# mattiaskvist/yolo-v1

Hardware: AMD Instinct MI355X
Metric: images/sec at 448x448, forward (YOLOv1Backbone + FC head) (higher is better)
Workload: dtype bf16; 1 GPU; BASELINE.json configs[1]: batch=64/GPU 448x448 forward-only, YOLOv1Backbone + FC head, 1xMI355X per rank; global_batch=64, per_gpu_batch=64, weights=random init (torch default, seed 0), parallelism=single

## Files before the change

include/yolo_hip.h:

```cpp
#ifndef YOLO_HIP_H
#define YOLO_HIP_H

#include <stddef.h>
#include <stdint.h>

#ifdef __cplusplus
extern "C" {
#endif

#define YOLO_HIP_ABI_VERSION 2

#define YOLO_E_ARG (-1)
#define YOLO_E_UNSUPPORTED (-2)

typedef void *yolo_stream_t;

int yolo_hip_abi_version(void);
const char *yolo_hip_last_error(void);
int yolo_debug_stamps(void *buf, int k_iter);
int yolo_stream_create(int low, yolo_stream_t *out);


int yolo_decode(const float *pred, int N, int S, int B, int C, double conf_thr,
                double *rec, int32_t *counts, yolo_stream_t stream);
// ... 52 lines not shown
#define YOLO_EPI_BIAS_LRELU 2
#define YOLO_EPI_MUL_DLRELU 3

#define YOLO_EPI_BIAS_ADD_LRELU 4

int yolo_igemm(const yolo_igemm_desc *d, const void *in_bf16, const void *w_bf16 ,
               const float *bias, const void *aux_bf16, void *out, yolo_stream_t stream);
int yolo_igemm_finish(const yolo_igemm_desc *d, const float *acc, const float *bias, const void *aux_bf16,
                      void *out_bf16, yolo_stream_t stream);

typedef struct yolo_wgrad_desc {
    int64_t P;
    int32_t dy_px_stride, x_px_stride;
    int32_t Cout, Cin;
    int32_t KH, KW, pad;
    int64_t x_row_stride;
    int32_t split;
    int32_t accumulate;
    int32_t variant;
    int32_t geo_W, geo_H, geo_img_slots, geo_row_slots, geo_px_slots, geo_slot0;
    double *dw_sumsq;
    float *slabs;
    int64_t slab_floats;
} yolo_wgrad_desc;

int yolo_wgrad_slab_floats(const yolo_wgrad_desc *d, long *floats);
int yolo_wgrad(const yolo_wgrad_desc *d, const void *x_bf16, const void *dy_bf16,
               float *dw_packed, float *db, yolo_stream_t stream);

typedef struct yolo_pool_desc {
    int32_t N, H, W, C;
    int32_t in_halo, out_halo;
} yolo_pool_desc;
int yolo_maxpool3s2_fwd(const yolo_pool_desc *d, const void *x_bf16, void *y_bf16, yolo_stream_t stream);
int yolo_maxpool3s2_bwd(const yolo_pool_desc *d, const void *x_bf16, const void *dy_bf16, void *dx_bf16, int dx_halo,
                        yolo_stream_t stream);
int yolo_maxpool2_fwd(const yolo_pool_desc *d, const void *x_bf16, void *y_bf16, yolo_stream_t stream);
int yolo_maxpool2_bwd_lrelu(const yolo_pool_desc *d, const void *yfull_bf16, const void *dpool_bf16,
                            float slope, void *dz_bf16, yolo_stream_t stream);
int yolo_maxpool2_bwd_codes(const yolo_pool_desc *d, const void *ypool_bf16, const void *codes_u16, const void *dpool_bf16,
                            float slope, void *dz_bf16, yolo_stream_t stream);


int yolo_nchw_f32_to_nhwc_bf16(const float *x, int N, int C, int H, int W, void *y, int Cpad,
                               int halo_lo, int halo_hi, yolo_stream_t stream);
int yolo_nhwc_bf16_to_nchw_f32(const void *x, int N, int C, int H, int W, int halo, float *y, yolo_stream_t stream);
int yolo_nhwc_bf16_to_nchw_bf16(const void *x, int N, int C, int H, int W, int halo, void *y, yolo_stream_t stream);

int yolo_pack_conv_weight(const float *w_oihw, int Cout, int Cin, int KH, int KW, int Cinp, int KWp,
                          void *w_fwd_bf16, void *w_dgrad_bf16, yolo_stream_t stream);
int yolo_pack_fc_weight(const float *w, int O, int C, int HW, void *w_fwd_bf16, void *w_t_bf16, yolo_stream_t stream);
int yolo_pack_fc_weight_blocked(const float *w, int O, long K, void *w_panels_bf16, yolo_stream_t stream);
int yolo_pack_fc_weight_blocked_hwc(const float *w, int O, int C, int HW, void *w_panels_bf16, yolo_stream_t stream);
int yolo_unpack_conv_wgrad(const float *dw_packed, int Cout, int Cin, int KH, int KW, int Cinp, int KWp,
                           float *dw_oihw, int accumulate, yolo_stream_t stream);
int yolo_conv_stem7_fwd(const void *x_nhwc4_bf16, const void *w_packed_bf16, const float *bias, int N, int Ho, int Wo,
                        long x_img_stride, int x_row_stride, float slope, int pool2, void *out_bf16,
                        long out_img_stride, int out_row_stride, int out_off, void *out_full_bf16,
                        long full_img_stride, int full_row_stride, int full_off, yolo_stream_t stream);
int yolo_conv_stem7_fwd_f32(const float *x_nchw_f32, const void *w_packed_bf16, const float *bias, int N, int H, int W, float slope,
                            int pool2, void *out_bf16, long out_img_stride, int out_row_stride, int out_off, void *out_full_bf16,
                            long full_img_stride, int full_row_stride, int full_off, yolo_stream_t stream);
int yolo_wgrad_stem7(const void *x_nhwc4_bf16, const void *dy_bf16, int N, int Ho, int Wo, long x_img_stride,
                     int x_row_stride, long dy_img_stride, int dy_row_stride, int dy_off, float *dw_oihw,
                     float *db, float *scratch, long scratch_elems, yolo_stream_t stream);
int yolo_wgrad_stem7_pooled(const void *x_nhwc4_bf16, const void *y_full_bf16, int N, int Ho, int Wo, long x_img_stride,
                            int x_row_stride, long y_img_stride, int y_row_stride, int y_off, const void *dpool_bf16,
                            long dp_img_stride, int dp_row_stride, int dp_off, float slope, float *dw_oihw, float *db,
                            float *scratch, long scratch_elems, yolo_stream_t stream);
int yolo_wgrad_stem7_codes(const void *x_nhwc4_bf16, const void *y_pooled_bf16, const void *codes_u16, int N, int Ho, int Wo,
                           long x_img_stride, int x_row_stride, const void *dpool_bf16, long dp_img_stride, int dp_row_stride,
                           int dp_off, float slope, float *dw_oihw, float *db, float *scratch, long scratch_elems,
                           yolo_stream_t stream);
#define YOLO_PACK_MAX 32
typedef struct yolo_conv_pack_item {
    const float *w;
    void *w_fwd_bf16;
    void *w_dgrad_bf16;
    int Cout, Cin, KH, KW;
} yolo_conv_pack_item;
typedef struct yolo_conv_unpack_item {
    const float *dw_packed;
    float *dw_oihw;
    int Cout, Cin, KH, KW;
} yolo_conv_unpack_item;
int yolo_pack_conv_weights_multi(const yolo_conv_pack_item *items, int count, yolo_stream_t stream);
int yolo_unpack_conv_wgrads_multi(const yolo_conv_unpack_item *items, int count, yolo_stream_t stream);
int yolo_im2col_rows(const void *x_bf16, long x_img_stride, int x_row_stride, int x_px_stride, int stride,
                     int KH, int seg, int N, int Ho, int Wo, int out_halo, void *xcol_bf16, yolo_stream_t stream);
int yolo_transpose_f32_to_bf16(const float *x, int R, int Ccols, void *y_bf16, int ld, yolo_stream_t stream);
int yolo_transpose_bf16(const void *x_bf16, int R, int Ccols, int ldx, void *y_bf16, int ldy, yolo_stream_t stream);
int yolo_fc_dgrad_to_nhwc(const float *dxT, int N, int C, int H, int W, int halo, const void *y_act_bf16,
                          float slope, void *g_bf16, yolo_stream_t stream);
int yolo_cast_f32_to_bf16(const float *x, long n, void *y_bf16, yolo_stream_t stream);
int yolo_cast_bf16_to_f32(const void *x_bf16, long n, float *y, yolo_stream_t stream);
int yolo_bias_lrelu_rows(const float *x, const float *bias, int R, int Ccols, float slope,
                         void *y_bf16, float *y_f32, yolo_stream_t stream);
int yolo_bias_lrelu_rows_slabs(const float *x, int slabs, const float *bias, int R, int Ccols, float slope,
                               void *y_bf16, float *y_f32, yolo_stream_t stream);

int yolo_scale_rows_to_bf16(const float *x, const unsigned char *mask, float scale, const void *act_bf16, float slope,
                            int R, int Cc, int ld, void *y_bf16, yolo_stream_t stream);
int yolo_dropout_bf16(const void *x_bf16, const unsigned char *mask, float scale, long n, void *y_bf16, yolo_stream_t stream);

int yolo_sumsq_f32(const float *g, long n, double *acc, yolo_stream_t stream);
int yolo_adam_step(float *p, const float *g, float *exp_avg, float *exp_avg_sq, long n, float lr, float beta1,
// ... 101 lines not shown
```

yolo-v1_amd/yolo/_hip.py:

```python

from __future__ import annotations

import ctypes
import os

import torch

_HERE = os.path.dirname(os.path.abspath(__file__))
LIB_PATH = os.environ.get("YOLO_HIP_LIB") or os.path.join(_HERE, "libyolo_hip.so")
_LIB = None

ABI_VERSION = 2
BN_ACC_REPLICAS = 16
c_int, c_long, c_float, c_double, c_void_p = ctypes.c_int, ctypes.c_long, ctypes.c_float, ctypes.c_double, ctypes.c_void_p


class IgemmDesc(ctypes.Structure):

    _fields_ = [
        ("N", ctypes.c_int32), ("Ho", ctypes.c_int32), ("Wo", ctypes.c_int32),
        ("in_img_stride", ctypes.c_int64),
        ("in_row_stride", ctypes.c_int32), ("in_px_stride", ctypes.c_int32), ("in_off", ctypes.c_int32),
        ("stride", ctypes.c_int32), ("KH", ctypes.c_int32), ("KW", ctypes.c_int32),
        ("tap_len", ctypes.c_int32), ("Cout", ctypes.c_int32),
# ... 68 lines not shown
                ("htab", c_void_p), ("vtab", c_void_p),
                ("hk", ctypes.c_int32), ("vk", ctypes.c_int32),
                ("n_ops", ctypes.c_int32), ("ops", ctypes.c_int32 * 3),
                ("brightness", ctypes.c_float), ("saturation", ctypes.c_float), ("hue_shift", ctypes.c_int32), ("reserved", ctypes.c_int32)]


AUG_BRIGHTNESS, AUG_SATURATION, AUG_HUE = 0, 1, 2
EPI_NONE, EPI_BIAS, EPI_BIAS_LRELU, EPI_MUL_DLRELU, EPI_BIAS_ADD_LRELU = 0, 1, 2, 3, 4
NMS_INFERENCE, NMS_METRICS = 0, 1

_SIGS = {
    "yolo_hip_abi_version": [],
    "yolo_debug_stamps": [c_void_p, c_int],
    "yolo_stream_create": [c_int, ctypes.POINTER(c_void_p)],
    "yolo_decode": [c_void_p, c_int, c_int, c_int, c_int, c_double, c_void_p, c_void_p, c_void_p],
    "yolo_decode_gt": [c_void_p, c_int, c_int, c_int, c_int, c_void_p, c_void_p, c_void_p],
    "yolo_nms": [c_void_p, c_void_p, c_int, c_int, c_double, c_int, c_void_p, c_void_p, c_void_p],
    "yolo_batchnorm_train_fwd": [c_void_p, c_int, c_int, c_int, c_int, c_int, c_void_p, c_void_p, c_double, c_double, c_void_p, c_void_p, c_void_p, c_int,
                                 c_int, c_void_p, c_void_p, c_void_p, c_int, c_void_p, c_int, c_void_p],
    "yolo_batchnorm_bwd": [c_void_p, c_int, c_void_p, c_int, c_void_p, c_int, c_int, c_int, c_int, c_int, c_void_p, c_void_p, c_void_p, ctypes.c_long, ctypes.c_long,
                           ctypes.c_long, ctypes.c_long, c_int, c_int, c_void_p, c_void_p, c_void_p, c_void_p, c_void_p],
    "yolo_map_match": [c_void_p, c_void_p, c_void_p, c_int, c_int, c_void_p, c_void_p, c_int, ctypes.POINTER(c_double), c_int, c_double, c_double, c_double,
                       c_void_p, c_void_p, c_void_p],
    "yolo_pairwise_iou": [c_void_p, c_int, c_void_p, c_int, c_int, c_void_p, c_void_p],
    "yolo_loss_fwd_bwd": [c_void_p, c_void_p, c_int, c_int, c_int, c_int, c_float, c_float, c_void_p, c_void_p, c_void_p, c_void_p],
    "yolo_loss_iou": [c_void_p, c_void_p, c_long, c_void_p, c_void_p],
    "yolo_igemm": [ctypes.POINTER(IgemmDesc), c_void_p, c_void_p, c_void_p, c_void_p, c_void_p, c_void_p],
    "yolo_igemm_finish": [ctypes.POINTER(IgemmDesc), c_void_p, c_void_p, c_void_p, c_void_p, c_void_p],
    "yolo_wgrad": [ctypes.POINTER(WgradDesc), c_void_p, c_void_p, c_void_p, c_void_p, c_void_p],
    "yolo_wgrad_slab_floats": [ctypes.POINTER(WgradDesc), ctypes.POINTER(ctypes.c_long)],
    "yolo_conv_stem7_fwd": [c_void_p, c_void_p, c_void_p, c_int, c_int, c_int, c_long, c_int, c_float, c_int, c_void_p, c_long, c_int, c_int, c_void_p, c_long,
                            c_int, c_int, c_void_p],
    "yolo_conv_stem7_fwd_f32": [c_void_p, c_void_p, c_void_p, c_int, c_int, c_int, c_float, c_int, c_void_p, c_long, c_int, c_int, c_void_p, c_long, c_int, c_int,
                                c_void_p],
    "yolo_wgrad_stem7": [c_void_p, c_void_p, c_int, c_int, c_int, c_long, c_int, c_long, c_int, c_int, c_void_p, c_void_p, c_void_p, c_long, c_void_p],
    "yolo_wgrad_stem7_pooled": [c_void_p, c_void_p, c_int, c_int, c_int, c_long, c_int, c_long, c_int, c_int, c_void_p, c_long, c_int, c_int, c_float, c_void_p,
                                c_void_p, c_void_p, c_long, c_void_p],
    "yolo_wgrad_stem7_codes": [c_void_p, c_void_p, c_void_p, c_int, c_int, c_int, c_long, c_int, c_void_p, c_long, c_int, c_int, c_float, c_void_p, c_void_p, c_void_p,
                               c_long, c_void_p],
    "yolo_maxpool3s2_fwd": [ctypes.POINTER(PoolDesc), c_void_p, c_void_p, c_void_p],
    "yolo_maxpool3s2_bwd": [ctypes.POINTER(PoolDesc), c_void_p, c_void_p, c_void_p, c_int, c_void_p],
    "yolo_maxpool2_fwd": [ctypes.POINTER(PoolDesc), c_void_p, c_void_p, c_void_p],
    "yolo_maxpool2_bwd_lrelu": [ctypes.POINTER(PoolDesc), c_void_p, c_void_p, c_float, c_void_p, c_void_p],
    "yolo_maxpool2_bwd_codes": [ctypes.POINTER(PoolDesc), c_void_p, c_void_p, c_void_p, c_float, c_void_p, c_void_p],
    "yolo_nchw_f32_to_nhwc_bf16": [c_void_p, c_int, c_int, c_int, c_int, c_void_p, c_int, c_int, c_int, c_void_p],
    "yolo_nhwc_bf16_to_nchw_f32": [c_void_p, c_int, c_int, c_int, c_int, c_int, c_void_p, c_void_p],
    "yolo_nhwc_bf16_to_nchw_bf16": [c_void_p, c_int, c_int, c_int, c_int, c_int, c_void_p, c_void_p],
    "yolo_scale_rows_to_bf16": [c_void_p, c_void_p, c_float, c_void_p, c_float, c_int, c_int, c_int, c_void_p, c_void_p],
    "yolo_dropout_bf16": [c_void_p, c_void_p, c_float, c_long, c_void_p, c_void_p],
    "yolo_pack_conv_weight": [c_void_p, c_int, c_int, c_int, c_int, c_int, c_int, c_void_p, c_void_p, c_void_p],
    "yolo_pack_fc_weight": [c_void_p, c_int, c_int, c_int, c_void_p, c_void_p, c_void_p],
    "yolo_pack_fc_weight_blocked": [c_void_p, c_int, c_long, c_void_p, c_void_p],
    "yolo_pack_fc_weight_blocked_hwc": [c_void_p, c_int, c_int, c_int, c_void_p, c_void_p],
    "yolo_unpack_conv_wgrad": [c_void_p, c_int, c_int, c_int, c_int, c_int, c_int, c_void_p, c_int, c_void_p],
    "yolo_im2col_rows": [c_void_p, c_long, c_int, c_int, c_int, c_int, c_int, c_int, c_int, c_int, c_int, c_void_p, c_void_p],
    "yolo_transpose_f32_to_bf16": [c_void_p, c_int, c_int, c_void_p, c_int, c_void_p],
    "yolo_transpose_bf16": [c_void_p, c_int, c_int, c_int, c_void_p, c_int, c_void_p],
    "yolo_fc_dgrad_to_nhwc": [c_void_p, c_int, c_int, c_int, c_int, c_int, c_void_p, c_float, c_void_p, c_void_p],
    "yolo_cast_f32_to_bf16": [c_void_p, c_long, c_void_p, c_void_p],
    "yolo_cast_bf16_to_f32": [c_void_p, c_long, c_void_p, c_void_p],
    "yolo_preprocess_u8": [c_void_p, c_int, c_int, c_int, c_int, c_int, c_void_p, c_void_p, c_int, c_void_p, c_void_p, c_int, c_void_p,
                           ctypes.POINTER(c_float), ctypes.POINTER(c_float), c_void_p, c_int, c_void_p, c_void_p],
    "yolo_augment_u8": [c_void_p, ctypes.c_int64, ctypes.POINTER(AugmentDesc), c_void_p, c_int, c_int, c_int, c_void_p, ctypes.c_int64,
                        ctypes.POINTER(c_float), ctypes.POINTER(c_float), c_void_p, c_int, c_void_p, c_void_p, c_void_p],
    "yolo_sumsq_f32": [c_void_p, c_long, c_void_p, c_void_p],
    "yolo_adam_step": [c_void_p, c_void_p, c_void_p, c_void_p, c_long, c_float, c_float, c_float, c_float, c_float, c_long, c_void_p, c_float, c_void_p, c_void_p],
    "yolo_clip_scale_f32": [c_void_p, c_long, c_void_p, c_float, c_void_p],
    "yolo_pack_conv_weights_multi": [ctypes.POINTER(ConvPackItem), c_int, c_void_p],
    "yolo_unpack_conv_wgrads_multi": [ctypes.POINTER(ConvUnpackItem), c_int, c_void_p],
    "yolo_sumsq_f32_multi": [c_void_p, c_void_p, c_int, c_void_p, c_void_p],
    "yolo_sumsq_fixed_slots": [ctypes.POINTER(c_long), c_int, ctypes.POINTER(c_long)],
    "yolo_sumsq_f32_fixed": [c_void_p, c_long, c_void_p, c_long, c_void_p, c_void_p],
    "yolo_sumsq_f32_multi_fixed": [c_void_p, c_void_p, c_int, c_void_p, c_long, c_void_p, c_void_p],
    "yolo_adam_step_multi": [ctypes.POINTER(AdamTensor), c_int, c_float, c_float, c_float, c_float, c_float, c_long, c_void_p, c_float, c_void_p, c_void_p],
    "yolo_adam_step_multi_bg": [ctypes.POINTER(AdamTensor), c_int, c_float, c_float, c_float, c_float, c_float, c_long, c_void_p, c_float, c_void_p, c_int, c_void_p],
    "yolo_sgd_step": [c_void_p, c_void_p, c_void_p, c_long, c_float, c_float, c_float, c_float, c_int, c_int, c_void_p, c_float, c_void_p, c_void_p, c_void_p],
    "yolo_sgd_step_multi": [ctypes.POINTER(SgdTensor), c_int, c_float, c_float, c_float, c_float, c_int, c_int, c_void_p, c_float, c_void_p, c_void_p],
    "yolo_sgd_step_multi_bg": [ctypes.POINTER(SgdTensor), c_int, c_float, c_float, c_float, c_float, c_int, c_int, c_void_p, c_float, c_void_p, c_int, c_void_p],
    "yolo_ema_update": [c_void_p, c_void_p, c_long, c_float, c_void_p, c_void_p],
    "yolo_ema_update_multi": [ctypes.POINTER(EmaTensor), c_int, c_float, c_void_p, c_void_p],
    "yolo_ema_update_multi_bg": [ctypes.POINTER(EmaTensor), c_int, c_float, c_void_p, c_int, c_void_p],
    "yolo_bias_lrelu_rows": [c_void_p, c_void_p, c_int, c_int, c_float, c_void_p, c_void_p, c_void_p],
    "yolo_bias_lrelu_rows_slabs": [c_void_p, c_int, c_void_p, c_int, c_int, c_float, c_void_p, c_void_p, c_void_p],
}


def available() -> bool:
    return os.path.exists(LIB_PATH)


def lib():
    global _LIB
    if _LIB is None:
        if not os.path.exists(LIB_PATH):
            raise RuntimeError(
                f"{LIB_PATH} not found: the gfx950 HIP library is not built (run `make -C yolo-v1_amd/csrc` or "
                "`python -c 'import __graft_entry__ as g; g.build()'`).  This package has no CPU/eager fallback for GPU tensors.")
        L = ctypes.CDLL(LIB_PATH)
        L.yolo_hip_abi_version.argtypes, L.yolo_hip_abi_version.restype = [], c_int
        if L.yolo_hip_abi_version() != ABI_VERSION:
            raise RuntimeError(f"{LIB_PATH} has ABI version {L.yolo_hip_abi_version()}, this package binds version {ABI_VERSION}: rebuild it "
                               "(`make -C yolo-v1_amd/csrc`)")
        for name, args in _SIGS.items():
            fn = getattr(L, name)
            fn.argtypes = args
            fn.restype = c_int
# ... 66 lines not shown
```

yolo-v1_amd/yolo/config.py:

```python

from __future__ import annotations

from dataclasses import dataclass, fields


@dataclass
class EngineConfig:
    TIMERS: list | None = None
    IGEMM_LAUNCHES: int = 0
    TUNE_LOG: list | None = None
    AUTOTUNE: bool = False
    TILE_HINT: int = 0
    TILE_PX: int = 0
    PLAN_TABLE: bool = True
    BORROW_PLANS: bool = True
    SMALL_SPLIT: bool = True
    PERSIST: bool = True
    BN_STATS_IN_CONV: bool = True
    STEM_KERNEL: bool = True
    STEM_POOL_BWD_FUSED: bool = True
    STRIDE2_CLASSES: bool = True
    STEM_F32_INPUT: bool = True
    FLATTEN_FREE: bool = True
    POOL_CODES: bool = True
    FUSE_POOL: bool = True
    FC_NORM_IN_WGRAD: int = 1 << 26
    WGRAD_STREAM: bool = True
    SIDE_LOW: bool = True
    WGRAD_SLABS: bool = False
    WGRAD_PIPE: bool = True
    WGRAD_CHOICE: object = None
    PLAN_TIMES: object = None
    TUNE_REPS: int = 1
    FC_WGRAD_SIDE: bool = True
    DETERMINISTIC: bool = False
    WGRAD_WIDE: bool = True


def _from_env(cfg: EngineConfig) -> EngineConfig:
    import os
    for f in fields(EngineConfig):
        v = os.environ.get("YOLO_AMD_" + f.name)
        if v is None:
            continue
        if f.type not in ("bool", "int"):
            raise ValueError(f"YOLO_AMD_{f.name}: only the bool / int switches can be set from the environment")
        setattr(cfg, f.name, bool(int(v)) if f.type == "bool" else int(v))
    return cfg


CONFIG = _from_env(EngineConfig())
SWITCHES = frozenset(f.name for f in fields(EngineConfig))
```

yolo-v1_amd/yolo/executor.py:

```python

from __future__ import annotations

import ctypes
from dataclasses import dataclass

import torch
import torch.nn as nn

from . import _hip
from ._hip import (EPI_BIAS, EPI_BIAS_LRELU, EPI_MUL_DLRELU, EPI_NONE, ConvPackItem, ConvUnpackItem, IgemmDesc, PoolDesc, WgradDesc, check, ptr)
from .config import CONFIG as CFG
from .plans import igemm_call
from .runtime import (RT, Act, _attach_wgrad_slabs, _EventSlot, _igemm, _on_side_stream, _round_up, _timed, desc_aux, igemm_desc, rows_desc,
                      stem_tiles_ok)


@dataclass
class Layer:
    kind: str
    name: str = ""
    Cout: int = 0
    Cin: int = 0
    K: int = 1
    stride: int = 1
    pad: int = 0
    lrelu: bool = False
    dropout: float = 0.0
    drop_mod: object = None
    weight: nn.Parameter | None = None
    bias: nn.Parameter | None = None
    first: bool = False
    Hin: int = 0
    Win: int = 0
    Hout: int = 0
    Wout: int = 0


class Plan:

    SLOPE = 0.1

    def __init__(self, layers: list[Layer], in_channels: int, input_is_image: bool, S: int | None = None):
        self.layers = layers
        self.in_channels = in_channels
        self.input_is_image = input_is_image
        self.params: list[nn.Parameter] = []
        for L in layers:
            if L.kind in ("conv", "fc"):
                self.params += [L.weight, L.bias]
        self._pf: dict[int, tuple] = {}
        self._pd: dict[int, tuple] = {}
        self._pfb: dict[int, tuple] = {}
        self._pd2: dict[int, tuple] = {}
        self._ws: dict[tuple, list] = {}
        self.grad_norm_sq: dict = {}
        self.debug_keep = False
        self.last = None
        self.arena = None
        self.arena_views: dict[int, tuple] = {}
        self.on_grad_ready = None
        self.on_backward_done = None
        self.on_stream_wait = None
        self.cfg = None
        self.params_ready = _EventSlot()
        self.owner = None

    @property
    def c(self):
        return self.cfg if self.cfg is not None else CFG

    def attach_grad_arena(self, device) -> torch.Tensor:
        order = [li for li in reversed(range(len(self.layers))) if self.layers[li].kind in ("conv", "fc")]
        off = 0
        wv, bv = {}, {}
        for li in order:
            n = self.layers[li].weight.numel()
            wv[li] = (off, off + n, _round_up(off + n, 64))
            off = _round_up(off + n, 64)
        self._arena_w_end = off
        for li in order:
            n = self.layers[li].bias.numel()
            bv[li] = (off, off + n)
            off = _round_up(off + n, 64)
        self.arena = torch.zeros(off, dtype=torch.float32, device=device)
        self.arena_views = {li: (self.arena[wv[li][0]:wv[li][1]].view_as(self.layers[li].weight),
                                 self.arena[bv[li][0]:bv[li][1]].view_as(self.layers[li].bias), wv[li][0], wv[li][2])
                            for li in order}
        return self.arena

    @staticmethod
    def _side_stream(dev) -> "torch.cuda.Stream":
        key = torch.device(dev).index
        if key not in RT._SIDE_STREAMS:
            RT._SIDE_STREAMS[key] = RT.STREAMS.side(dev, CFG.SIDE_LOW)
        return RT._SIDE_STREAMS[key]

    def _layer_done(self, li: int):
        if self.arena is not None and self.on_grad_ready is not None:
            _, _, a, b = self.arena_views[li]
            self.on_grad_ready(a, b)

    @staticmethod
    def from_modules(mods, in_channels: int, input_is_image: bool) -> "Plan":
        layers: list[Layer] = []
        i = 0
# ... 105 lines not shown
                self._pf[li] = (key, wf)
                return wf, None
            if wf is None:
                wf = torch.empty((L.Cout, L.K, L.K, L.Cin), dtype=torch.bfloat16, device=dev)
            if need_dgrad and wd is None:
                wd = torch.empty((L.Cin, L.K, L.K, L.Cout), dtype=torch.bfloat16, device=dev)
            check(RT.lib().yolo_pack_conv_weight(ptr(wsrc), L.Cout, L.Cin, L.K, L.K, L.Cin, L.K, None if ok_f else ptr(wf),
                                              ptr(wd) if (need_dgrad and not ok_d) else None, RT.stream()), "pack_conv_weight")
        else:
            if not ok_f:
                if wf is None:
                    wf = torch.empty((L.Cout, L.Cin), dtype=torch.bfloat16, device=dev)
                check(RT.lib().yolo_cast_f32_to_bf16(ptr(wsrc), wsrc.numel(), ptr(wf), RT.stream()), "cast fc weight")
            if need_dgrad and not ok_d:
                ld = _round_up(L.Cout, 32)
                if wd is None:
                    wd = torch.zeros((L.Cin, ld), dtype=torch.bfloat16, device=dev)
                check(RT.lib().yolo_transpose_f32_to_bf16(ptr(wsrc), L.Cout, L.Cin, ptr(wd), ld, RT.stream()), "transpose")
        self._pf[li] = (key, wf)
        if need_dgrad:
            self._pd[li] = (key, wd)
            return wf, wd
        return wf, (wd if ok_d else None)

    def _stride2_panels(self, li: int, wdg: torch.Tensor) -> dict:
        L = self.layers[li]
        key = self._wkey(L.weight)
        hit = self._pd2.get(li)
        if hit is not None and hit[0] == key:
            return hit[1]
        sel = {0: slice(1, 2), 1: slice(0, 3, 2)}
        panels = {}
        for py in (0, 1):
            for px in (0, 1):
                panels[(py, px)] = wdg[:, sel[py], sel[px], :].contiguous()
        self._pd2[li] = (key, panels)
        return panels

    def _pack_fc_blocked(self, li: int, hwc=None):
        L = self.layers[li]
        key = (self._wkey(L.weight), hwc)
        hit = self._pfb.get(li)
        if hit is not None and hit[0] == key:
            return hit[1]
        wsrc = self._src(L)
        wb = hit[1] if hit is not None else torch.empty((_round_up(L.Cout, 128) * L.Cin,), dtype=torch.bfloat16, device=L.weight.device)
        if hwc is not None:
            check(RT.lib().yolo_pack_fc_weight_blocked_hwc(ptr(wsrc), L.Cout, hwc[0], hwc[1], ptr(wb), RT.stream()), "pack_fc_blocked_hwc")
        else:
            check(RT.lib().yolo_pack_fc_weight_blocked(ptr(wsrc), L.Cout, L.Cin, ptr(wb), RT.stream()), "pack_fc_blocked")
        self._pfb[li] = (key, wb)
        return wb

    def fc_biases(self):
        return [L.bias for L in self.layers if L.kind == "fc" and L.bias is not None and L.bias.is_cuda]

    def bf16_shadows(self):
        out = []
        for li, L in enumerate(self.layers):
            if L.kind != "fc" or not L.weight.is_cuda:
                continue
            wf, _ = self._pack(li, False)

            def fresh(p, li=li, wf=wf):
                self._pf[li] = (self._wkey(p), wf)
            out.append((L.weight, wf, fresh))
        return out

    def _workspace(self, N: int, x_shape, device, train: bool):
        key = (N, tuple(x_shape[1:]), str(device), train)
        pool = self._ws.setdefault(key, [])
        if pool:
            ws = pool.pop()
            self._apply_geom(ws)
            return key, ws
        ws = {"acts": [], "grads": {}, "misc": {}, "geom": {}}
        C, H, W = x_shape[1], x_shape[2], x_shape[3]
        if self.layers and self.layers[0].kind == "conv" and self.layers[0].first:
            a = Act(N, H, W, 4, 3, device)
        else:
            a = Act(N, H, W, C, 1, device)
        ws["in"] = a
        cur = a
        flat = None
        for li, L in enumerate(self.layers):
            if L.kind == "conv":
                L.Hin, L.Win = cur.H, cur.W
                L.Hout = (cur.H + 2 * L.pad - L.K) // L.stride + 1
                L.Wout = (cur.W + 2 * L.pad - L.K) // L.stride + 1
                dense = (not train and self.c.FLATTEN_FREE and li + 2 < len(self.layers) and self.layers[li + 1].kind == "flatten"
                         and self.layers[li + 2].kind == "fc" and L.Cout % 8 == 0 and (L.Cout * L.Hout * L.Wout) % 64 == 0)
                cur = Act(N, L.Hout, L.Wout, L.Cout, 0 if dense else 1, device)
            elif L.kind == "pool":
                L.Hin, L.Win = cur.H, cur.W
                cur = Act(N, cur.H // 2, cur.W // 2, cur.C, 1, device)
            elif L.kind == "flatten":
                flat = torch.empty((N, cur.C * cur.H * cur.W), dtype=torch.bfloat16, device=device)
                cur = flat
            elif L.kind == "fc":
                feat = flat.shape[1] if (flat is not None and cur is flat) else None
                if feat is not None and feat != L.Cin:
                    raise RuntimeError(f"mat1 and mat2 shapes cannot be multiplied ({N}x{feat} and {L.Cin}x{L.Cout}): input of "
                                       f"{tuple(x_shape[2:])} pixels does not match the Linear layer behind nn.Flatten")
                cur = None
            ws["acts"].append(cur)
            ws["geom"][li] = (L.Hin, L.Win, L.Hout, L.Wout)
# ... 112 lines not shown
            codes = self._codes(f.ws, li, dst) if f.codes_mode else None
            if codes is not None:
                d.pool2, aux = 3, ptr(codes)
            else:
                d.pool2, aux = 2, full.p
                desc_aux(d, full)
        with _timed(f"conv{li}" + ("+pool" if (fuse or dual) else ""), "igemm", 2.0 * N * L.Hout * L.Wout * L.Cout * L.Cin * L.K * L.K):
            igemm_call(d, cur.p, ptr(wf), ptr(b), aux, dst.p, f.st, f"igemm conv{li}")
        f.cur = dst
        return 2 if (fuse or dual) else 1

    def _fwd_stem(self, f, li: int, wf, b, fuse: bool, dual: bool) -> int:
        L, N, cur = self.layers[li], f.N, f.cur
        full = f.ws["acts"][li]
        dst = f.ws["acts"][li + 1] if (fuse or dual) else full
        codes = self._codes(f.ws, li, dst) if (dual and f.codes_mode) else None
        slope = self.SLOPE if L.lrelu else 1.0
        if codes is not None:
            pool2, second = 3, (ptr(codes), 0, 0, 0)
        elif dual:
            pool2, second = 1, (full.p, full.img_stride, full.row_stride, full.interior_off())
        else:
            pool2, second = (1 if fuse else 0), (None, 0, 0, 0)
        out = (dst.p, dst.img_stride, dst.row_stride, dst.interior_off())
        with _timed(f"conv{li}" + ("+pool" if (fuse or dual) else ""), "stem", 2.0 * N * L.Hout * L.Wout * L.Cout * L.Cin * L.K * L.K):
            if f.x32 is not None and li == 0:
                x = f.x32
                check(f.lib.yolo_conv_stem7_fwd_f32(ptr(x), ptr(wf), ptr(b), N, x.shape[2], x.shape[3], slope, pool2, *out, *second, f.st), "conv_stem7_fwd_f32")
            else:
                check(f.lib.yolo_conv_stem7_fwd(cur.p, ptr(wf), ptr(b), N, L.Hout, L.Wout, cur.img_stride, cur.row_stride, slope, pool2, *out, *second, f.st),
                      "conv_stem7_fwd")
        f.cur = dst
        return 2 if (fuse or dual) else 1

    def _fwd_pool(self, f, li: int) -> int:
        cur, nxt = f.cur, f.ws["acts"][li]
        pd = PoolDesc(f.N, cur.H, cur.W, cur.C, cur.halo, nxt.halo)
        with _timed(f"pool{li}", "maxpool2_fwd"):
            check(f.lib.yolo_maxpool2_fwd(ctypes.byref(pd), cur.p, nxt.p, f.st), "maxpool")
        f.cur = nxt
        return 1

    def _fwd_flatten(self, f, li: int) -> int:
        cur = f.cur
        if not f.train and isinstance(cur, Act) and cur.halo == 0 and cur.halo_hi == 0 and self.c.FLATTEN_FREE:
            f.hwc = (cur.C, cur.H * cur.W)
            f.cur = cur.t.view(f.N, -1)
            return 1
        nxt = f.ws["acts"][li]
        check(f.lib.yolo_nhwc_bf16_to_nchw_bf16(cur.p, f.N, cur.C, cur.H, cur.W, cur.halo, ptr(nxt), f.st), "flatten")
        f.cur = nxt
        return 1

    def _fwd_fc(self, f, li: int) -> int:
        L, N, dev, L_, st = self.layers[li], f.N, f.dev, f.lib, f.st
        self.params_ready.wait(dev)
        if f.train:
            wf, _ = self._pack(li, False)
        else:
            wf = self._pack_fc_blocked(li, f.hwc)
            f.hwc = None
        xin = f.cur
        K = L.Cin
        d = rows_desc(N, xin.shape[1], K, L.Cout)
        d.slope, d.out_fp32 = self.SLOPE, 1
        d.w_blocked = 0 if f.train else 1
        last = (li == len(self.layers) - 1)
        nk = K // 64
        splits = max(1, min(32 if d.w_blocked else 48, nk // 16)) if K >= 4096 else 1
        b = L.bias.detach()
        if splits > 1:
            acc = RT._splitk_scratch(splits * N * L.Cout, zero=False)
            d.epilogue, d.split_k, d.split_slabs = EPI_NONE, splits, 1
            with _timed(f"fc{li}", "igemm", 2.0 * N * L.Cout * L.Cin):
                _igemm(L_, d, ptr(xin), ptr(wf), None, None, ptr(acc), st, f"igemm fc{li}")
            yb = torch.empty((N, L.Cout), dtype=torch.bfloat16, device=dev) if not last else None
            yf = torch.empty((N, L.Cout), dtype=torch.float32, device=dev) if last else None
            check(L_.yolo_bias_lrelu_rows_slabs(ptr(acc), splits, ptr(b), N, L.Cout, self.SLOPE if L.lrelu else 1.0, ptr(yb), ptr(yf), st),
                  "bias_lrelu_rows")
        else:
            yf = torch.empty((N, L.Cout), dtype=torch.float32, device=dev)
            d.epilogue, d.split_k = (EPI_BIAS_LRELU if L.lrelu else EPI_BIAS), 1
            with _timed(f"fc{li}", "igemm", 2.0 * N * L.Cout * L.Cin):
                _igemm(L_, d, ptr(xin), ptr(wf), ptr(b), None, ptr(yf), st, f"igemm fc{li}")
            yb = None
            if not last:
                yb = torch.empty((N, L.Cout), dtype=torch.bfloat16, device=dev)
                check(L_.yolo_cast_f32_to_bf16(ptr(yf), yf.numel(), ptr(yb), st), "cast")
        mask = None
        if L.drop_mod is not None:
            L.dropout = float(L.drop_mod.p)
        f.cur = yb
        if not last and L.dropout > 0 and f.drop_training:
            mask = (torch.rand((N, L.Cout), device=dev) >= L.dropout).to(torch.uint8)
            f.cur = torch.empty_like(yb)
            check(L_.yolo_dropout_bf16(ptr(yb), ptr(mask), 1.0 / max(1.0 - L.dropout, 1e-12) if L.dropout < 1.0 else 0.0, yb.numel(), ptr(f.cur), st), "dropout")
        f.fc_saved[li] = (xin, yb, mask)
        if last:
            f.out = yf
        return 1

    @staticmethod
    def _codes(ws, li: int, pooled: Act) -> torch.Tensor:
        c = ws["misc"].get(("codes", li))
        if c is None:
            c = torch.empty(pooled.t.numel() // 8, dtype=torch.int16, device=pooled.t.device)
            ws["misc"][("codes", li)] = c
        ws["codes"].add(li)
        return c

    @staticmethod
    def _misc(ws, key, make):
        buf = ws["misc"].get(key)
        if buf is None:
            buf = ws["misc"][key] = make()
        return buf

    def _grad_buf(self, ws, li: int, N, dev) -> Act:
        g = ws["grads"].get(li)
        if g is None:
            L = self.layers[li]
            if L.stride == 1 or L.first:
                g = Act(N, L.Hout, L.Wout, L.Cout, 1, dev)
            else:
                g = Act(N, L.Hin, L.Win, L.Cout, 1, dev)
            ws["grads"][li] = g
        return g

    @staticmethod
    def _wgrad_desc(L: Layer, g: Act, xin: Act, N: int) -> WgradDesc:
        px = N * L.Hout * L.Wout
        deep = (L.Cout >= 512 and L.Cin >= 256 and px >= 40000) or (L.Cout >= 1024 and L.Cin >= 1024 and px >= 12000)
        variant = 5 if (CFG.WGRAD_PIPE and L.K == 3 and L.stride == 1 and deep) else 0
        flat = False
        if CFG.WGRAD_PIPE and CFG.WGRAD_WIDE and L.K == 3 and L.stride == 1:
            if (deep and L.Cin < 1024) or (L.Cin == 64 and L.Cout >= 192 and px >= 500000):
                variant = 6
                flat = L.Hout >= 56 and L.Wout >= 56
        geo_ok = L.Hout >= 2 and L.Wout >= 2
        geo = variant >= 5 or (geo_ok and (L.stride > 1 or g.Hp * g.Wp >= 1.12 * L.Hout * L.Wout))
        choice = CFG.WGRAD_CHOICE.get((N, L.Hout, L.Wout, L.Cout, L.Cin, L.K, L.stride)) if CFG.WGRAD_CHOICE else None
# ... 338 lines not shown
```

Measured before the change: 24340 images/s.

## Add dedicated streaming FC-head kernels with a new weight-panel layout for inference

Adds a new packed weight layout for the FC layers and two specialized kernels. The first is a split-K streaming kernel for large K that keeps weight panels in registers, uses nontemporal loads and double-buffers activations in LDS. The second is a small-K kernel that reduces across waves and fuses bias and leaky ReLU. Inference FC layers now take this path when the shape constraints hold, replacing the generic igemm, since this head (batch 64, huge K) is bound by weight bandwidth. It adds a new packing cache entry and relies on splits being tuned to the CU count.

```diff
diff --git a/include/yolo_hip.h b/include/yolo_hip.h
--- a/include/yolo_hip.h
+++ b/include/yolo_hip.h
@@ -128,6 +128,11 @@
 int yolo_pack_fc_weight(const float *w, int O, int C, int HW, void *w_fwd_bf16, void *w_t_bf16, yolo_stream_t stream);
 int yolo_pack_fc_weight_blocked(const float *w, int O, long K, void *w_panels_bf16, yolo_stream_t stream);
 int yolo_pack_fc_weight_blocked_hwc(const float *w, int O, int C, int HW, void *w_panels_bf16, yolo_stream_t stream);
+int yolo_pack_fc_weight_stream(const float *w, int O, int C, int HW, void *w_stream_bf16, yolo_stream_t stream);
+int yolo_fc_stream(const void *x_bf16, long ldx, int N, const void *w_stream_bf16, int O, long K, int splits, float *slabs,
+                   yolo_stream_t stream);
+int yolo_fc_small(const void *x_bf16, long ldx, int N, const void *w_stream_bf16, int O, long K, const float *bias, float slope,
+                  void *y_bf16, float *y_f32, yolo_stream_t stream);
 int yolo_unpack_conv_wgrad(const float *dw_packed, int Cout, int Cin, int KH, int KW, int Cinp, int KWp,
                            float *dw_oihw, int accumulate, yolo_stream_t stream);
 int yolo_conv_stem7_fwd(const void *x_nhwc4_bf16, const void *w_packed_bf16, const float *bias, int N, int Ho, int Wo,
diff --git a/yolo-v1_amd/csrc/fc_head.hip b/yolo-v1_amd/csrc/fc_head.hip
--- /dev/null
+++ b/yolo-v1_amd/csrc/fc_head.hip
@@ -0,0 +1,272 @@
+#include "common.h"
+#include "igemm_common.h"
+
+namespace yolo {
+
+__global__ void pack_fc_stream_kernel(const float *__restrict__ w, int O, int C, int HW, long total, uint4 *__restrict__ wp)
+{
+    const long idx = (long)blockIdx.x * blockDim.x + threadIdx.x;
+    if (idx >= total) return;
+    const long K = (long)C * HW;
+    const long ng = (O + 63) / 64;
+    const int lane = (int)(idx & 63);
+    const int sub = (int)((idx >> 6) & 3), half = (int)((idx >> 8) & 1);
+    const long bg = idx >> 9;
+    const long g = bg % ng, kb = bg / ng;
+    const long o = g * 64 + sub * 16 + (lane & 15);
+    const long k = kb * 64 + half * 32 + (lane >> 4) * 8;
+    unsigned short h[8];
+    if (o < O) {
+        const long hw = k / C, c = k % C;
+        const float *src = w + o * K + c * HW + hw;
+#pragma unroll
+        for (int j = 0; j < 8; ++j) h[j] = f32_to_bf16(src[(long)j * HW]);
+    } else {
+#pragma unroll
+        for (int j = 0; j < 8; ++j) h[j] = 0;
+    }
+    uint4 v;
+    v.x = h[0] | ((unsigned)h[1] << 16);
+    v.y = h[2] | ((unsigned)h[3] << 16);
+    v.z = h[4] | ((unsigned)h[5] << 16);
+    v.w = h[6] | ((unsigned)h[7] << 16);
+    wp[idx] = v;
+}
+
+typedef __attribute__((ext_vector_type(4))) unsigned u32x4;
+__device__ __forceinline__ bf16x8 as_bf16x8(const u32x4 &v) { return __builtin_bit_cast(bf16x8, v); }
+
+constexpr int FCS_CHUNK_BLOCKS = 4;
+constexpr int FCS_CHUNK_STEPS = FCS_CHUNK_BLOCKS * 2;
+
+template <int RT>
+__global__ __launch_bounds__(256, 1) void fc_stream_kernel(const bf16_t *__restrict__ x, long ldx, int N, const u32x4 *__restrict__ wp, int O, int nkb,
+                                                           int splits, float *__restrict__ slabs)
+{
+    __shared__ u32x4 xs[2][FCS_CHUNK_STEPS][RT][64];
+    const int tid = threadIdx.x, lane = tid & 63, wave = tid >> 6;
+    const int s = blockIdx.x % splits;
+    const int g = (blockIdx.x / splits) * 4 + wave;
+    const bool active = g < (O + 63) / 64;
+    const int kb0 = (int)((long)s * nkb / splits), kb1 = (int)((long)(s + 1) * nkb / splits);
+    const int nb = kb1 - kb0;
+    const long ng = (O + 63) / 64;
+    const u32x4 *wg = wp + ((long)kb0 * ng + (active ? g : 0)) * 512 + lane;
+
+    const int sk16 = tid & 31;
+    const int srow = tid >> 5;
+    const int sdst = (sk16 >> 2) * RT * 64 + (sk16 & 3) * 16;
+    u32x4 xr[2 * RT];
+    auto stage_load = [&](int chunk) {
+        const int kstep = min(chunk * FCS_CHUNK_STEPS + (sk16 >> 2), 2 * nb - 1);
+        const bf16_t *px = x + (2L * kb0 + kstep) * 32 + (sk16 & 3) * 8;
+#pragma unroll
+        for (int q = 0; q < 2 * RT; ++q) xr[q] = *reinterpret_cast<const u32x4 *>(px + (long)min(srow + 8 * q, N - 1) * ldx);
+    };
+    auto stage_store = [&](int buf) {
+        u32x4 *dst = &xs[buf][0][0][0] + sdst;
+#pragma unroll
+        for (int q = 0; q < 2 * RT; ++q) {
+            const int n = srow + 8 * q;
+            dst[(n >> 4) * 64 + (n & 15)] = xr[q];
+        }
+    };
+
+    f32x4 acc[4][RT];
+#pragma unroll
+    for (int i = 0; i < 4; ++i)
+#pragma unroll
+        for (int r = 0; r < RT; ++r) acc[i][r] = f32x4{0.f, 0.f, 0.f, 0.f};
+
+    u32x4 w0[8], w1[8], w2[8], w3[8];
+    auto load_w = [&](u32x4(&w)[8], int b) {
+        const u32x4 *p = wg + (long)(b < nb ? b : nb - 1) * ng * 512;
+#pragma unroll
+        for (int i = 0; i < 8; ++i) w[i] = __builtin_nontemporal_load(p + i * 64);
+    };
+    auto compute = [&](const u32x4(&w)[8], int buf, int b) {
+        const u32x4 *xb = &xs[buf][(b & (FCS_CHUNK_BLOCKS - 1)) * 2][0][0] + lane;
+#pragma unroll
+        for (int h = 0; h < 2; ++h) {
+            bf16x8 xf[RT];
+#pragma unroll
+            for (int r = 0; r < RT; ++r) xf[r] = as_bf16x8(xb[(h * RT + r) * 64]);
+#pragma unroll
+            for (int i = 0; i < 4; ++i)
+#pragma unroll
+                for (int r = 0; r < RT; ++r)
+                    acc[i][r] = __builtin_amdgcn_mfma_f32_16x16x32_bf16(as_bf16x8(w[h * 4 + i]), xf[r], acc[i][r], 0, 0, 0);
+        }
+    };
+
+    load_w(w0, 0);
+    load_w(w1, 1);
+    load_w(w2, 2);
+    stage_load(0);
+    stage_store(0);
+    int b = 0;
+    for (; b + FCS_CHUNK_BLOCKS <= nb; b += FCS_CHUNK_BLOCKS) {
+        const int buf = (b / FCS_CHUNK_BLOCKS) & 1;
+        __syncthreads();
+        stage_load(b / FCS_CHUNK_BLOCKS + 1);
+        load_w(w3, b + 3);
+        __builtin_amdgcn_sched_barrier(0);
+        compute(w0, buf, b);
+        __builtin_amdgcn_sched_barrier(0);
+        load_w(w0, b + 4);
+        __builtin_amdgcn_sched_barrier(0);
+        compute(w1, buf, b + 1);
+        __builtin_amdgcn_sched_barrier(0);
+        load_w(w1, b + 5);
+        __builtin_amdgcn_sched_barrier(0);
+        compute(w2, buf, b + 2);
+        __builtin_amdgcn_sched_barrier(0);
+        load_w(w2, b + 6);
+        __builtin_amdgcn_sched_barrier(0);
+        compute(w3, buf, b + 3);
+        __builtin_amdgcn_sched_barrier(0);
+        stage_store(buf ^ 1);
+    }
+    if (b < nb) {
+        const int buf = (b / FCS_CHUNK_BLOCKS) & 1;
+        __syncthreads();
+        compute(w0, buf, b);
+        if (b + 1 < nb) compute(w1, buf, b + 1);
+        if (b + 2 < nb) compute(w2, buf, b + 2);
+    }
+
+    if (!active) return;
+    float *out = slabs + (long)s * N * O;
+#pragma unroll
+    for (int r = 0; r < RT; ++r) {
+        const int n = r * 16 + (lane & 15);
+        if (n >= N) continue;
+#pragma unroll
+        for (int i = 0; i < 4; ++i) {
+            const int o = g * 64 + i * 16 + (lane >> 4) * 4;
+            float *p = out + (long)n * O + o;
+            if ((O & 3) == 0 && o + 3 < O) {
+                *reinterpret_cast<f32x4 *>(p) = acc[i][r];
+            } else {
+#pragma unroll
+                for (int j = 0; j < 4; ++j)
+                    if (o + j < O) p[j] = acc[i][r][j];
+            }
+        }
+    }
+}
+
+constexpr int FCM_WAVES = 8;
+constexpr int FCM_UNROLL = 8;
+
+template <int RT>
+__global__ __launch_bounds__(64 * FCM_WAVES) void fc_small_kernel(const bf16_t *__restrict__ x, long ldx, int N, const u32x4 *__restrict__ wp, int O, int nks,
+                                                                  const float *__restrict__ bias, float slope, bf16_t *__restrict__ yb, float *__restrict__ yf)
+{
+    __shared__ f32x4 red[FCM_WAVES][RT][64];
+    const int tid = threadIdx.x, lane = tid & 63, wave = tid >> 6;
+    const int o16 = blockIdx.x;
+    const long ng = (O + 63) / 64;
+    const u32x4 *wg = wp + ((long)(o16 >> 2) * 8 + (o16 & 3)) * 64 + lane;
+    auto wk = [&](int ks) { return ((long)(ks >> 1) * ng * 8 + (ks & 1) * 4) * 64; };
+    const bf16_t *xp[RT];
+#pragma unroll
+    for (int r = 0; r < RT; ++r) xp[r] = x + (long)min(r * 16 + (lane & 15), N - 1) * ldx + (lane >> 4) * 8;
+    f32x4 acc[RT];
+#pragma unroll
+    for (int r = 0; r < RT; ++r) acc[r] = f32x4{0.f, 0.f, 0.f, 0.f};
+
+    int ks = wave;
+    for (; ks + (FCM_UNROLL - 1) * FCM_WAVES < nks; ks += FCM_UNROLL * FCM_WAVES) {
+        u32x4 wv[FCM_UNROLL], xv[FCM_UNROLL][RT];
+#pragma unroll
+        for (int u = 0; u < FCM_UNROLL; ++u) {
+            wv[u] = wg[wk(ks + u * FCM_WAVES)];
+#pragma unroll
+            for (int r = 0; r < RT; ++r) xv[u][r] = *reinterpret_cast<const u32x4 *>(xp[r] + (long)(ks + u * FCM_WAVES) * 32);
+        }
+        __builtin_amdgcn_sched_barrier(0);
+#pragma unroll
+        for (int u = 0; u < FCM_UNROLL; ++u)
+#pragma unroll
+            for (int r = 0; r < RT; ++r) acc[r] = __builtin_amdgcn_mfma_f32_16x16x32_bf16(as_bf16x8(wv[u]), as_bf16x8(xv[u][r]), acc[r], 0, 0, 0);
+    }
+    for (; ks < nks; ks += FCM_WAVES) {
+        const u32x4 wv = wg[wk(ks)];
+#pragma unroll
+        for (int r = 0; r < RT; ++r)
+            acc[r] = __builtin_amdgcn_mfma_f32_16x16x32_bf16(as_bf16x8(wv), as_bf16x8(*reinterpret_cast<const u32x4 *>(xp[r] + (long)ks * 32)), acc[r], 0, 0, 0);
+    }
+#pragma unroll
+    for (int r = 0; r < RT; ++r) red[wave][r][lane] = acc[r];
+    __syncthreads();
+    if (tid >= RT * 64) return;
+    const int r = tid >> 6;
+    f32x4 v = red[0][r][lane];
+#pragma unroll
+    for (int w = 1; w < FCM_WAVES; ++w) v += red[w][r][lane];
+    const int n = r * 16 + (lane & 15);
+    if (n >= N) return;
+#pragma unroll
+    for (int j = 0; j < 4; ++j) {
+        const int o = o16 * 16 + (lane >> 4) * 4 + j;
+        if (o >= O) continue;
+        float t = v[j] + (bias ? bias[o] : 0.0f);
+        t = t > 0.0f ? t : t * slope;
+        if (yf) yf[(long)n * O + o] = t;
+        if (yb) yb[(long)n * O + o] = f32_to_bf16(t);
+    }
+}
+
+static bool fc_rows_ok(const void *x, long ldx, int N, long K) { return N >= 1 && N <= 64 && K >= 64 && (K & 63) == 0 && ldx >= K && (ldx & 7) == 0 && ((uintptr_t)x & 15) == 0; }
+
+}
+
+using namespace yolo;
+
+YOLO_API int yolo_pack_fc_weight_stream(const float *w, int O, int C, int HW, void *wp, yolo_stream_t stream)
+{
+    if (!w || !wp || O <= 0 || C <= 0 || HW <= 0 || (C & 7) || (((long)C * HW) & 63))
+        return fail(YOLO_E_ARG, "yolo_pack_fc_weight_stream: bad argument (C must be a multiple of 8, C * HW of 64)");
+    const long total = (long)((O + 63) / 64) * ((long)C * HW / 32) * 256;
+    hipLaunchKernelGGL(pack_fc_stream_kernel, dim3((unsigned)((total + 255) / 256)), dim3(256), 0, STRM(stream), w, O, C, HW, total, (uint4 *)wp);
+    return check_launch("yolo_pack_fc_weight_stream");
+}
+
+YOLO_API int yolo_fc_stream(const void *x, long ldx, int N, const void *wp, int O, long K, int splits, float *slabs, yolo_stream_t stream)
+{
+    if (!x || !wp || !slabs || O <= 0 || splits < 1) return fail(YOLO_E_ARG, "yolo_fc_stream: bad argument");
+    if (!fc_rows_ok(x, ldx, N, K) || K > (1L << 30)) return fail(YOLO_E_UNSUPPORTED, "yolo_fc_stream: at most 64 rows, K a multiple of 64, x rows 16-B aligned");
+    if (splits > K / 64 || ((uintptr_t)slabs & 15)) return fail(YOLO_E_UNSUPPORTED, "yolo_fc_stream: more K ranges than 64-deep blocks, or slabs not 16-B aligned");
+    const int nkb = (int)(K / 64);
+    const long grid = (long)splits * ((O + 255) / 256);
+    if (grid > 0x7fffffffL) return fail(YOLO_E_UNSUPPORTED, "yolo_fc_stream: grid too large");
+    const bf16_t *xp = (const bf16_t *)x;
+    const u32x4 *w4 = (const u32x4 *)wp;
+    const dim3 gr((unsigned)grid), bl(256);
+    switch ((N + 15) / 16) {
+    case 1: hipLaunchKernelGGL(fc_stream_kernel<1>, gr, bl, 0, STRM(stream), xp, ldx, N, w4, O, nkb, splits, slabs); break;
+    case 2: hipLaunchKernelGGL(fc_stream_kernel<2>, gr, bl, 0, STRM(stream), xp, ldx, N, w4, O, nkb, splits, slabs); break;
+    case 3: hipLaunchKernelGGL(fc_stream_kernel<3>, gr, bl, 0, STRM(stream), xp, ldx, N, w4, O, nkb, splits, slabs); break;
+    default: hipLaunchKernelGGL(fc_stream_kernel<4>, gr, bl, 0, STRM(stream), xp, ldx, N, w4, O, nkb, splits, slabs); break;
+    }
+    return check_launch("yolo_fc_stream");
+}
+
+YOLO_API int yolo_fc_small(const void *x, long ldx, int N, const void *wp, int O, long K, const float *bias, float slope, void *yb, float *yf,
+                           yolo_stream_t stream)
+{
+    if (!x || !wp || (!yb && !yf) || O <= 0) return fail(YOLO_E_ARG, "yolo_fc_small: bad argument");
+    if (!fc_rows_ok(x, ldx, N, K) || K > (1L << 24)) return fail(YOLO_E_UNSUPPORTED, "yolo_fc_small: at most 64 rows, K a multiple of 64, x rows 16-B aligned");
+    const int nks = (int)(K / 32);
+    const bf16_t *xp = (const bf16_t *)x;
+    const u32x4 *w4 = (const u32x4 *)wp;
+    const dim3 gr((unsigned)((O + 15) / 16)), bl(64 * FCM_WAVES);
+    switch ((N + 15) / 16) {
+    case 1: hipLaunchKernelGGL(fc_small_kernel<1>, gr, bl, 0, STRM(stream), xp, ldx, N, w4, O, nks, bias, slope, (bf16_t *)yb, yf); break;
+    case 2: hipLaunchKernelGGL(fc_small_kernel<2>, gr, bl, 0, STRM(stream), xp, ldx, N, w4, O, nks, bias, slope, (bf16_t *)yb, yf); break;
+    case 3: hipLaunchKernelGGL(fc_small_kernel<3>, gr, bl, 0, STRM(stream), xp, ldx, N, w4, O, nks, bias, slope, (bf16_t *)yb, yf); break;
+    default: hipLaunchKernelGGL(fc_small_kernel<4>, gr, bl, 0, STRM(stream), xp, ldx, N, w4, O, nks, bias, slope, (bf16_t *)yb, yf); break;
+    }
+    return check_launch("yolo_fc_small");
+}
diff --git a/yolo-v1_amd/yolo/_hip.py b/yolo-v1_amd/yolo/_hip.py
--- a/yolo-v1_amd/yolo/_hip.py
+++ b/yolo-v1_amd/yolo/_hip.py
@@ -144,6 +144,9 @@
     "yolo_pack_fc_weight": [c_void_p, c_int, c_int, c_int, c_void_p, c_void_p, c_void_p],
     "yolo_pack_fc_weight_blocked": [c_void_p, c_int, c_long, c_void_p, c_void_p],
     "yolo_pack_fc_weight_blocked_hwc": [c_void_p, c_int, c_int, c_int, c_void_p, c_void_p],
+    "yolo_pack_fc_weight_stream": [c_void_p, c_int, c_int, c_int, c_void_p, c_void_p],
+    "yolo_fc_stream": [c_void_p, c_long, c_int, c_void_p, c_int, c_long, c_int, c_void_p, c_void_p],
+    "yolo_fc_small": [c_void_p, c_long, c_int, c_void_p, c_int, c_long, c_void_p, c_float, c_void_p, c_void_p, c_void_p],
     "yolo_unpack_conv_wgrad": [c_void_p, c_int, c_int, c_int, c_int, c_int, c_int, c_void_p, c_int, c_void_p],
     "yolo_im2col_rows": [c_void_p, c_long, c_int, c_int, c_int, c_int, c_int, c_int, c_int, c_int, c_int, c_void_p, c_void_p],
     "yolo_transpose_f32_to_bf16": [c_void_p, c_int, c_int, c_void_p, c_int, c_void_p],
diff --git a/yolo-v1_amd/yolo/config.py b/yolo-v1_amd/yolo/config.py
--- a/yolo-v1_amd/yolo/config.py
+++ b/yolo-v1_amd/yolo/config.py
@@ -22,6 +22,7 @@
     STRIDE2_CLASSES: bool = True
     STEM_F32_INPUT: bool = True
     FLATTEN_FREE: bool = True
+    FC_HEAD: bool = True
     POOL_CODES: bool = True
     FUSE_POOL: bool = True
     FC_NORM_IN_WGRAD: int = 1 << 26
diff --git a/yolo-v1_amd/yolo/executor.py b/yolo-v1_amd/yolo/executor.py
--- a/yolo-v1_amd/yolo/executor.py
+++ b/yolo-v1_amd/yolo/executor.py
@@ -50,7 +50,7 @@
                 self.params += [L.weight, L.bias]
         self._pf: dict[int, tuple] = {}
         self._pd: dict[int, tuple] = {}
-        self._pfb: dict[int, tuple] = {}
+        self._pfb: dict = {}
         self._pd2: dict[int, tuple] = {}
         self._ws: dict[tuple, list] = {}
         self.grad_norm_sq: dict = {}
@@ -262,6 +262,19 @@
         self._pfb[li] = (key, wb)
         return wb
 
+    def _pack_fc_stream(self, li: int, hwc=None):
+        L = self.layers[li]
+        key = (self._wkey(L.weight), hwc)
+        hit = self._pfb.get((li, "stream"))
+        if hit is not None and hit[0] == key:
+            return hit[1]
+        wsrc = self._src(L)
+        wp = hit[1] if hit is not None else torch.empty((_round_up(L.Cout, 64) * L.Cin,), dtype=torch.bfloat16, device=L.weight.device)
+        C, HW = hwc if hwc is not None else (L.Cin, 1)
+        check(RT.lib().yolo_pack_fc_weight_stream(ptr(wsrc), L.Cout, C, HW, ptr(wp), RT.stream()), "pack_fc_stream")
+        self._pfb[(li, "stream")] = (key, wp)
+        return wp
+
     def fc_biases(self):
         return [L.bias for L in self.layers if L.kind == "fc" and L.bias is not None and L.bias.is_cuda]
 
@@ -480,9 +493,61 @@
         f.cur = nxt
         return 1
 
+    _CUS: dict = {}
+
+    @classmethod
+    def _cu_count(cls, dev) -> int:
+        if dev.type != "cuda":
+            return 0
+        key = dev.index if dev.index is not None else torch.cuda.current_device()
+        if key not in cls._CUS:
+            cls._CUS[key] = int(torch.cuda.get_device_properties(key).multi_processor_count)
+        return cls._CUS[key]
+
+    @staticmethod
+    def _fc_stream_splits(Cout: int, K: int, cus: int = 256) -> int:
+        groups = (Cout + 255) // 256
+        s = min(-(-cus // groups), K // 64 // 8)
+        return max(1, s - s % 8 if s >= 8 else s)
+
+    def _fc_head(self, f, li: int, last: bool):
+        L, N, L_, st = self.layers[li], f.N, f.lib, f.st
+        xin, K = f.cur, L.Cin
+        ld = xin.shape[1]
+        cus = self._cu_count(f.dev)
+        if not cus:
+            return None
+        if N > 64 or K < 4096 or K % 64 or ld % 8 or xin.data_ptr() % 16 or (f.hwc is not None and f.hwc[0] % 8):
+            return None
+        wp = self._pack_fc_stream(li, f.hwc)
+        b = L.bias.detach()
+        slope = self.SLOPE if L.lrelu else 1.0
+        yb = torch.empty((N, L.Cout), dtype=torch.bfloat16, device=f.dev) if not last else None
+        yf = torch.empty((N, L.Cout), dtype=torch.float32, device=f.dev) if last else None
+        try:
+            if K > 4096:
+                splits = self._fc_stream_splits(L.Cout, K, cus)
+                acc = RT._splitk_scratch(splits * N * L.Cout, zero=False)
+                with _timed(f"fc{li}", "igemm", 2.0 * N * L.Cout * K):
+                    CFG.IGEMM_LAUNCHES += 1
+                    check(L_.yolo_fc_stream(ptr(xin), ld, N, ptr(wp), L.Cout, K, splits, ptr(acc), st), f"fc_stream fc{li}")
+                check(L_.yolo_bias_lrelu_rows_slabs(ptr(acc), splits, ptr(b), N, L.Cout, slope, ptr(yb), ptr(yf), st), "bias_lrelu_rows")
+            else:
+                with _timed(f"fc{li}", "igemm", 2.0 * N * L.Cout * K):
+                    CFG.IGEMM_LAUNCHES += 1
+                    check(L_.yolo_fc_small(ptr(xin), ld, N, ptr(wp), L.Cout, K, ptr(b), slope, ptr(yb), ptr(yf), st), f"fc_small fc{li}")
+        except _hip.HipUnsupported:
+            return None
+        f.hwc = None
+        return yb, yf
+
     def _fwd_fc(self, f, li: int) -> int:
         L, N, dev, L_, st = self.layers[li], f.N, f.dev, f.lib, f.st
         self.params_ready.wait(dev)
+        last = (li == len(self.layers) - 1)
+        head = self._fc_head(f, li, last) if not f.train and self.c.FC_HEAD else None
+        if head is not None:
+            return self._fc_finish(f, li, last, f.cur, *head)
         if f.train:
             wf, _ = self._pack(li, False)
         else:
@@ -493,7 +558,6 @@
         d = rows_desc(N, xin.shape[1], K, L.Cout)
         d.slope, d.out_fp32 = self.SLOPE, 1
         d.w_blocked = 0 if f.train else 1
-        last = (li == len(self.layers) - 1)
         nk = K // 64
         splits = max(1, min(32 if d.w_blocked else 48, nk // 16)) if K >= 4096 else 1
         b = L.bias.detach()
@@ -515,6 +579,10 @@
             if not last:
                 yb = torch.empty((N, L.Cout), dtype=torch.bfloat16, device=dev)
                 check(L_.yolo_cast_f32_to_bf16(ptr(yf), yf.numel(), ptr(yb), st), "cast")
+        return self._fc_finish(f, li, last, xin, yb, yf)
+
+    def _fc_finish(self, f, li: int, last: bool, xin, yb, yf) -> int:
+        L, N, dev, L_, st = self.layers[li], f.N, f.dev, f.lib, f.st
         mask = None
         if L.drop_mod is not None:
             L.dropout = float(L.drop_mod.p)
```

Result: no change. 24460 images/s (median of 6 runs) (+0.5%).
